# ntnu-arl/aerial_gym_simulator

Hardware: AMD Instinct MI355X
Metric: env-steps/sec at N_envs=8192 per GPU (dynamics-only) (higher is better)
Workload: dtype f32; 1 GPU; base_quadrotor position_setpoint_task, lee_position_control, empty_env, 1 sub-step/step (BASELINE configs[1]); num_envs_per_gpu=8192, num_envs_total=8192, rng=sync-free (device Philox4x32-10)

## Files before the change

### aerial_gym_simulator_amd/csrc/agx_dyn_position_step.h

```cpp
#pragma once

namespace agx {
#ifdef AGX_STEP_STAMPS
constexpr int kStampBlocks = 1024, kStampWords = 8;
__device__ unsigned long long g_step_stamps[kStampBlocks * 2 * kStampWords];
AGX_DEV void step_stamp(int k) {
  const unsigned long long t = k < 6 ? (unsigned long long)clock64() : (unsigned long long)wall_clock64();
  if ((threadIdx.x & 63u) == 0u && blockIdx.x < (unsigned)kStampBlocks)
    g_step_stamps[((size_t)blockIdx.x * 2 + (threadIdx.x >> 6)) * kStampWords + k] = t;
}
#define AGX_STAMP(k) step_stamp(k)
#define AGX_STAMP_ARRIVED(k) do { __builtin_amdgcn_s_waitcnt(0); step_stamp(k); } while (0)
#else
#define AGX_STAMP(k) do { } while (0)
#define AGX_STAMP_ARRIVED(k) do { } while (0)
#endif

AGX_DEV unsigned proof_key(float x) { return x >= 0.0f ? __float_as_uint(x) : 0x7FC00000u; }

__host__ __device__ inline unsigned proof_witness_bit(int episode_len, int reset_on_collision, int steps, float dist, float speed, float dt,
                                                      float vmax, float dv) {
  const int k = episode_len - steps + 1;
  if (k < 1 || k > AGX_PROOF_HORIZON || !(dist == dist) || !(speed == speed)) return 0u;
  bool w = k == 1 || !reset_on_collision;
  if (!w) {
    const float m = (float)(k - 1);
    const float travel = m * dt * fminf(vmax, speed + m * dv);
    w = dist + (travel * 1.01f + 1.0e-3f) < 8.0f;
  }
  return w ? (1u << k) : 0u;
}

template <bool MAX>
AGX_DEV unsigned wave_reduce_dpp(unsigned x) {
#define AGX_RED(ctrl)                                                                        \
  {                                                                                           \
    const unsigned y_ = (unsigned)__builtin_amdgcn_mov_dpp((int)x, (ctrl), 0xF, 0xF, true);   \
    x = MAX ? max(x, y_) : (x | y_);                                                          \
  }
  AGX_RED(0xB1)
  AGX_RED(0x4E)
  AGX_RED(0x124)
  AGX_RED(0x128)
#undef AGX_RED
  const unsigned r0 = (unsigned)__builtin_amdgcn_readlane((int)x, 0), r1 = (unsigned)__builtin_amdgcn_readlane((int)x, 16);
  const unsigned r2 = (unsigned)__builtin_amdgcn_readlane((int)x, 32), r3 = (unsigned)__builtin_amdgcn_readlane((int)x, 48);
  return MAX ? max(max(r0, r1), max(r2, r3)) : ((r0 | r1) | (r2 | r3));
}

AGX_DEV void proof_store_slot(const AgxTaskArgs &T, const AgxEnvBuffers &B, int wb, int nb, bool reset, unsigned horizon, int steps,
                              float dist, float speed) {
  const unsigned ar = wave_reduce_dpp<false>(reset ? 1u : 0u), hz = wave_reduce_dpp<false>(horizon);
  const unsigned ms = wave_reduce_dpp<true>((unsigned)max(steps, 0)), db = wave_reduce_dpp<true>(proof_key(dist));
  const unsigned vb = wave_reduce_dpp<true>(proof_key(speed));
  if ((threadIdx.x & 63u) == 0u) {
    uint4 *slot = reinterpret_cast<uint4 *>(T.proof_slots + ((size_t)(B.step_counter & 1) * nb + wb) * AGX_PROOF_SLOT_WORDS);
    slot[0] = make_uint4(((unsigned)B.step_counter + 1u) & 0x7FFFFFFFu, ar | (T.proof_mode == AGX_STEP_ANY ? 2u : 0u), hz, ms);
    slot[1] = make_uint4(db, vb, 0u, 0u);
  }
}

AGX_DEV void proof_fold_publish(const AgxTaskArgs &T, const AgxEnvBuffers &B, int nb) {
  const int lane = (int)(threadIdx.x & 63u);
  const uint32_t *bank = T.proof_slots + (size_t)((B.step_counter & 1) ^ 1) * nb * AGX_PROOF_SLOT_WORDS;
  unsigned t_and = 0x7FFFFFFFu, t_or = 0u, fl = 0u, hz = 0u, ms = 0u, db = 0u, vb = 0u;
  for (int b = lane; b < nb; b += 64) {
    const uint4 s0 = reinterpret_cast<const uint4 *>(bank + (size_t)b * AGX_PROOF_SLOT_WORDS)[0];
    const uint4 s1 = reinterpret_cast<const uint4 *>(bank + (size_t)b * AGX_PROOF_SLOT_WORDS)[1];
    t_and &= s0.x; t_or |= s0.x; fl |= s0.y; hz |= s0.z;
    ms = max(ms, s0.w); db = max(db, s1.x); vb = max(vb, s1.y);
  }
#pragma unroll
  for (int off = 32; off > 0; off >>= 1) {
    t_and &= (unsigned)__shfl_xor((int)t_and, off);
    t_or |= (unsigned)__shfl_xor((int)t_or, off);
    fl |= (unsigned)__shfl_xor((int)fl, off);
    hz |= (unsigned)__shfl_xor((int)hz, off);
    ms = max(ms, (unsigned)__shfl_xor((int)ms, off));
    db = max(db, (unsigned)__shfl_xor((int)db, off));
    vb = max(vb, (unsigned)__shfl_xor((int)vb, off));
  }
  if (lane != 0) return;
  const unsigned tag = t_and == t_or ? t_or : 0u;
  if (tag != 0u && (fl & 2u) && !(fl & 1u)) atomicAdd(T.proof_violation, 1u);
  uint32_t *h = T.proof_record;
  __hip_atomic_store(h + 7, tag, __ATOMIC_RELAXED, __HIP_MEMORY_SCOPE_SYSTEM);
  __builtin_amdgcn_fence(__ATOMIC_RELEASE, "wavefront");
  __builtin_amdgcn_s_waitcnt(0);
  __hip_atomic_store(h + 1, hz, __ATOMIC_RELAXED, __HIP_MEMORY_SCOPE_SYSTEM);
  __hip_atomic_store(h + 2, ms, __ATOMIC_RELAXED, __HIP_MEMORY_SCOPE_SYSTEM);
  __hip_atomic_store(h + 3, db, __ATOMIC_RELAXED, __HIP_MEMORY_SCOPE_SYSTEM);
  __hip_atomic_store(h + 4, vb, __ATOMIC_RELAXED, __HIP_MEMORY_SCOPE_SYSTEM);
  __hip_atomic_store(h + 5, fl, __ATOMIC_RELAXED, __HIP_MEMORY_SCOPE_SYSTEM);
  __builtin_amdgcn_fence(__ATOMIC_RELEASE, "wavefront");
  __builtin_amdgcn_s_waitcnt(0);
  __hip_atomic_store(h + 0, tag, __ATOMIC_RELAXED, __HIP_MEMORY_SCOPE_SYSTEM);
}

struct StepHandoff {
  float p[64], q[64], v[64], w[64];
  int reset[64];
};
template <int MODE>
AGX_DEV void position_step_quad(const AgxRobotParams &P0, const AgxEnvBuffers &B0, int n, const float *actions_in,
                                const AgxTaskArgs &T0, float *obs, StepHandoff *H) {
  constexpr bool FUSED = MODE != AGX_STEP_TWO;
  const int tid = threadIdx.x;
  AGX_STAMP(0); AGX_STAMP(6);
  AgxRobotParams P = P0;
  AgxEnvBuffers B = B0;
  AgxTaskArgs T = T0;
#define AGX_STEP_WAVE_ARGS(X)                                                                                                        \
  X(B, state) X(B, actions) X(B, prev_actions) X(B, motor_thrust) X(B, motor_kT) X(B, motor_tau_inc) X(B, motor_tau_dec)  \
  X(B, gains) X(B, wrench_cmd) X(B, crashes) X(B, truncations) X(B, sim_steps) X(B, reset_mask) X(B, reset_flag) X(B, flag_parity)    \
  X(B, step_counter) X(B, body_force)                                                                                                  \
  X(P, dt) X(P, dt_over_6) X(P, mass) X(P, min_thrust) X(P, max_thrust) X(P, max_rate) X(P, linear_damping) X(P, angular_damping)     \
  X(P, max_linear_velocity) X(P, max_angular_velocity) X(P, tau_inc_uniform) X(P, tau_dec_uniform)                                    \
  X(T, episode_len) X(T, target) X(T, reward) X(T, proof_slots) X(T, proof_violation) X(T, proof_dv)
  AGX_STEP_WAVE_ARGS(AGX_ARG_READ)
  AGX_ARG_READ(B, derived) AGX_ARG_READ(B, push_world)
  AGX_ARG_READ(P, root_link_mode) AGX_ARG_READ(P, use_rps) AGX_ARG_READ(P, use_discrete_approximation) AGX_ARG_READ(P, integration_rk4)
  AGX_ARG_READ(T, reset_on_collision) AGX_ARG_READ(T, kind) AGX_ARG_READ(T, proof_mode)
  const int grid_blocks = (int)gridDim.x;
  __builtin_amdgcn_sched_barrier(0);
  int env_blocks = grid_blocks - 1;
  int sw = (P_root_link_mode != 0 ? 1 : 0) | (P_use_rps != 0 ? 2 : 0) | (P_use_discrete_approximation != 0 ? 4 : 0) |
           (P_integration_rk4 != 0 ? 8 : 0) | (T_reset_on_collision != 0 ? 16 : 0) | ((T_kind & 0xFF) << 8) | ((T_proof_mode & 0xFF) << 16);
  arg_pin(n); arg_pin(actions_in);
  if (MODE == AGX_STEP_NONE) arg_pin(obs);
  AGX_STEP_WAVE_ARGS(AGX_ARG_PIN)
  if (MODE != AGX_STEP_ANY) { AGX_ARG_PIN(B, derived) }
  if (!FUSED) { AGX_ARG_PIN(B, push_world) }
  arg_pin(env_blocks);
#undef AGX_STEP_WAVE_ARGS
  arg_pin(sw);
  P.root_link_mode = sw & 1; P.use_rps = sw & 2; P.use_discrete_approximation = sw & 4; P.integration_rk4 = sw & 8;
  T.reset_on_collision = sw & 16; T.kind = (sw >> 8) & 0xFF; T.proof_mode = (sw >> 16) & 0xFF;
  const bool proof = T.proof_slots != nullptr;
  if (proof && blockIdx.x == 0) {
    proof_fold_publish(T0, B0, (int)gridDim.x - 1);
    AGX_STAMP(5); AGX_STAMP(7);
    return;
  }
  const int wb = (int)blockIdx.x - (proof ? 1 : 0);
  const int l = tid & 3, l3 = l < 3 ? l : 2;
  const int i = wb * 16 + (tid >> 2);
  const unsigned ol = ((unsigned)l * (unsigned)n + (unsigned)i) * 4u, ol3 = ((unsigned)l3 * (unsigned)n + (unsigned)i) * 4u;
  const bool valid = i < n;
  bool reset = false;
  if (FUSED && wb == 0 && tid == 0) B.reset_flag[B.flag_parity ^ 1] = 0;
  const bool push = !FUSED && wb == 0 && B.push_world > 0;
  uint32_t push_peek = 0u;
  if (__builtin_expect(push, false)) {
    push_publish_previous(B0);
    push_peek = push_wait_peek(B0);
  }
  float p = 0.0f, q = 0.0f, v = 0.0f, w = 0.0f, tgt = 0.0f, vbody = 0.0f, wbody = 0.0f;
  int steps = 0;
  float proof_dist = 0.0f, proof_speed = 0.0f;
  unsigned horizon = 0u;
  float u[1] = {0.0f}, a_in = 0.0f, a_old = 0.0f, fz = 0.0f, torque = 0.0f, dist = 0.0f;
  QuadDerived d{};
  bool crashed = false, trunc = false;
  AGX_STAMP(1);
  if (valid) {
    p = AGX_QAT(B.state, 0, ol3); q = AGX_QAT(B.state, 3, ol); v = AGX_QAT(B.state, 7, ol3); w = AGX_QAT(B.state, 10, ol3);
    u[0] = AGX_QAT(B.motor_thrust, 0, ol);
    float kT[1] = {1.0f}, tinc[1] = {P.tau_inc_uniform}, tdec[1] = {P.tau_dec_uniform};
    if (P.use_rps) kT[0] = AGX_QAT(B.motor_kT, 0, ol);
    if (B.motor_tau_inc) tinc[0] = AGX_QAT(B.motor_tau_inc, 0, ol);
    if (B.motor_tau_dec) tdec[0] = AGX_QAT(B.motor_tau_dec, 0, ol);
    a_in = actions_in[(size_t)i * 4 + l];
    a_old = AGX_QAT(B.actions, 0, ol);
    float kp = P0.gains_uniform[0 + l3], kv = P0.gains_uniform[3 + l3], kr = P0.gains_uniform[6 + l3], kw = P0.gains_uniform[9 + l3];
    if (B.gains) {
      kp = gain_load(&AGX_QAT(B.gains, 0, ol3)); kv = gain_load(&AGX_QAT(B.gains, 3, ol3));
      kr = gain_load(&AGX_QAT(B.gains, 6, ol3)); kw = gain_load(&AGX_QAT(B.gains, 9, ol3));
    }
    const int steps_in = B.sim_steps[i];
    tgt = T.kind == AGX_TASK_POSITION ? AGX_QAT(T.target, 0, ol3) : 0.0f;
    const QuadConsts<4> C = load_quad_consts<4>(P0, P, l, l3);
    AGX_STAMP_ARRIVED(2);

    const float a = clamp_minmax(a_in, -10.0f, 10.0f);
    float sy_sp, cy_sp;
    d = update_states_quad(q, v, w, q4::bc<3>(a), sy_sp, cy_sp);
    const float pe = a - p;
    const float ve = 0.0f - v;
    const float acc = kp * pe + kv * ve;
    const float f = (acc - C.grav) * C.mass;
    fz = quad_thrust_along_body_z(q, f, l);
    const float qd = quad_desired_orientation_pos_vel_sc(f, sy_sp, cy_sp, l);
    torque = quad_body_torque<true>(C, q, qd, d.wbody, 0.0f, kr, kw, l);

    float fb, tb;
    quad_allocate<4>(P, C, l == 2 ? fz : 0.0f, torque, u, kT, tinc, tdec, fb, tb);
    if (B.body_force && l < 3) AGX_QAT(B.body_force, 0, ol) = fb;
    quad_integrate(P, C, p, q, v, w, fb, tb, l);

    steps = steps_in + 1;
    if (T.kind == AGX_TASK_POSITION) {
      const float pe_t = q4::quat_apply(q4::conj(d.qveh), tgt - p);
      dist = q4::norm3(pe_t);
      if (dist > 8.0f) crashed = true;
      trunc = steps > T.episode_len;
      reset = (crashed && T.reset_on_collision) || trunc;
    }
  }
  AGX_STAMP(3);
  if (MODE == AGX_STEP_ANY) {
    H->p[tid] = p; H->q[tid] = q; H->v[tid] = v; H->w[tid] = w;
    H->reset[tid] = reset ? 1 : 0;
    __syncthreads();
  }
  AGX_STAMP(4);
  if (valid) {
    float rew = 0.0f;
    if (T.kind == AGX_TASK_POSITION) {
      const float ex = exp_cw((l == 0 ? -8.0f : -4.0f) * dist * dist);
      const float pos_reward = 3.0f * q4::bc<0>(ex) + 2.0f * q4::bc<1>(ex);
      const float dist_reward = (20.0f - dist) / 40.0f;
      const float axis_z = l == 2 ? 1.0f : 0.0f;
      const float up = q4::bc<2>(q4::quat_rotate(q, axis_z));
      const float tilt = fabsf(1.0f - up);
      const float spin = q4::norm3(d.wbody);
      const float quo = (1.0f / (l == 0 ? 0.1f + tilt * tilt : 1.0f + spin * spin)) * (l == 0 ? 0.2f : 3.0f);
      const float up_reward = q4::bc<0>(quo);
      const float ang_reward = q4::bc<1>(quo);
      float total = pos_reward + dist_reward + pos_reward * (up_reward + ang_reward);
      total = 1.0f * total;
      if (crashed) total = -20.0f;
      rew = total;
      proof_dist = dist;
    }
    if (proof) {
// ... 95 lines not shown
  float tgt = 0.0f;
  AGX_STAMP(1);
  if (valid) {
    steps_in = B.sim_steps[i];
    if (B.episode_count) ep = B.episode_count[i];
    tgt = T.kind == AGX_TASK_POSITION ? AGX_QAT(T.target, 0, ol3) : 0.0f;
  }
  AGX_STAMP_ARRIVED(2);
  const bool early = valid && T.kind == AGX_TASK_POSITION && steps_in + 1 > T.episode_len;
  ResetValues<4> V{};
  if (vote(early) != 0ull) {
    ResetDraws<4> D{};
    wave_reset_draws<4>(R, B.env_index_base + i, ep, early && l == 0, D);
    V = reset_env_values<4>(P, R, D);
  }
  AGX_STAMP(3);
  __syncthreads();
  AGX_STAMP(4);
  float p = H->p[lane], q = H->q[lane], v = H->v[lane], w = H->w[lane];
  const bool mine = H->reset[lane] != 0;
  const bool late = mine && !early;
  if (vote(late) != 0ull) {
    ResetDraws<4> D{};
    wave_reset_draws<4>(R, B.env_index_base + i, ep, late && l == 0, D);
    const ResetValues<4> V2 = reset_env_values<4>(P, R, D);
    if (late) V = V2;
  }
  if (vote(mine) != 0ull) {
    if (mine && l == 0) reset_env_store<4>(P, B, n, R, i, ep, V);
    const EnvState &s = V.s;
    const float npv = q4::by_lane(l3, q4::bc<0>(s.p.x), q4::bc<0>(s.p.y), q4::bc<0>(s.p.z));
    const float nq = q4::by_lane(l, q4::bc<0>(s.q.x), q4::bc<0>(s.q.y), q4::bc<0>(s.q.z), q4::bc<0>(s.q.w));
    const float nv = q4::by_lane(l3, q4::bc<0>(s.v.x), q4::bc<0>(s.v.y), q4::bc<0>(s.v.z));
    const float nw = q4::by_lane(l3, q4::bc<0>(s.w.x), q4::bc<0>(s.w.y), q4::bc<0>(s.w.z));
    p = mine ? npv : p; q = mine ? nq : q; v = mine ? nv : v; w = mine ? nw : w;
  }
  const QuadDerived d2 = update_states_quad(q, v, w);
  if (valid) {
    if (l < 3) {
      AGX_QAT(B.derived, 0, ol) = d2.euler;
      AGX_QAT(B.derived, 7, ol) = d2.vveh;
      AGX_QAT(B.derived, 10, ol) = d2.vbody;
      AGX_QAT(B.derived, 13, ol) = d2.wbody;
    }
    AGX_QAT(B.derived, 3, ol) = d2.qveh;
    float *o = obs + (size_t)i * 13;
    const float e = tgt - p;
    if (l < 3) { o[l] = e; o[7 + l] = d2.vbody; o[10 + l] = d2.wbody; }
    o[3 + l] = q;
  }
  AGX_STAMP(5); AGX_STAMP(7);
}

__global__ void __launch_bounds__(64, 1)
    k_env_step_quad_position(AgxRobotParams P, AgxEnvBuffers B, int n, const float *__restrict__ actions_in, AgxTaskArgs T) {
  position_step_quad<AGX_STEP_TWO>(P, B, n, actions_in, T, nullptr, nullptr);
}

template <int MODE>
__global__ void __launch_bounds__(MODE == AGX_STEP_ANY ? 128 : 64, 1)
    k_position_step_fused(AgxRobotParams P, AgxEnvBuffers B, int n, const float *__restrict__ actions_in, AgxTaskArgs T, AgxResetArgs R,
                          float *__restrict__ obs) {
  if constexpr (MODE == AGX_STEP_ANY) {
    __shared__ StepHandoff H;
    if (__builtin_amdgcn_readfirstlane((int)(threadIdx.x >> 6)) == 0) position_step_quad<MODE>(P, B, n, actions_in, T, obs, &H);
    else position_step_helper(P, B, n, T, R, obs, &H);
  } else {
    position_step_quad<MODE>(P, B, n, actions_in, T, obs, nullptr);
  }
}

#ifdef AGX_STEP_STAMPS
}
extern "C" int agx_debug_step_stamps(unsigned long long *out, int blocks) {
  if (blocks < 0 || blocks > agx::kStampBlocks) return -1;
  return (int)hipMemcpyFromSymbol(out, HIP_SYMBOL(agx::g_step_stamps), sizeof(unsigned long long) * 2 * agx::kStampWords * (size_t)blocks);
}
namespace agx {
#endif
}

extern "C" float agx_step_proof_dv(const AgxRobotParams *P) {
  if (!P || !(P->mass > 0.0f)) return INFINITY;
  const int M = P->num_motors;
  const float *wmap = P->root_link_mode != 0 ? P->alloc : P->wrench_map;
  float col = 0.0f;
  for (int j = 0; j < M; ++j) col += sqrtf(wmap[j] * wmap[j] + wmap[M + j] * wmap[M + j] + wmap[2 * M + j] * wmap[2 * M + j]);
  const float g = sqrtf(P->gravity[0] * P->gravity[0] + P->gravity[1] * P->gravity[1] + P->gravity[2] * P->gravity[2]);
  return (col * fmaxf(fabsf(P->max_thrust), fabsf(P->min_thrust)) / P->mass + g) * P->dt * 1.1f;
}

extern "C" float agx_step_proof_travel(int m, float speed, float dt, float vmax, float dv, int per_env) {
  if (m <= 0) return 0.0f;
  float travel = 0.0f;
  if (per_env) {
    travel = (float)m * dt * fminf(vmax, speed + (float)m * dv);
  } else {
    float v = speed;
    for (int k = 0; k < m; ++k) {
      v = fminf(v + dv, vmax);
      travel += v * dt;
    }
  }
  return travel * 1.01f + 1.0e-3f;
}

extern "C" uint32_t agx_step_proof_witness_bit(int episode_len, int reset_on_collision, int steps, float dist, float speed, float dt,
                                               float max_linear_velocity, float dv) {
  return proof_witness_bit(episode_len, reset_on_collision, steps, dist, speed, dt, max_linear_velocity, dv);
}

extern "C" int agx_step_proof_decide(const uint32_t *record, const AgxStepProofQuery *q, int32_t *reason) {
  int32_t why = AGX_PROOF_PROVED;
  int mode = AGX_STEP_TWO;
  if (!record || !q) {
    why = AGX_PROOF_OFF;
  } else {
    volatile const uint32_t *h = record;
    const uint32_t end = h[0];
    __atomic_thread_fence(__ATOMIC_ACQUIRE);
    const uint32_t hz = h[1], ms = h[2], db = h[3], vb = h[4], fl = h[5];
    __atomic_thread_fence(__ATOMIC_ACQUIRE);
    const uint32_t begin = h[7];
    const uint32_t k = (q->now_tag - end) & 0x7FFFFFFFu;
    float dist, speed;
    memcpy(&dist, &db, 4);
    memcpy(&speed, &vb, 4);
    if (end != begin) why = AGX_PROOF_TORN;
    else if (end == 0u) why = AGX_PROOF_NO_RECORD;
    else if (((end - q->min_tag) & 0x7FFFFFFFu) >= 0x40000000u) why = AGX_PROOF_VOID;
    else if (k == 0u || k > 64u) why = AGX_PROOF_TAG;
    else if (k <= AGX_PROOF_HORIZON && ((hz >> k) & 1u)) mode = AGX_STEP_ANY;
    else if (fl & 1u) why = AGX_PROOF_RESET_NO_WITNESS;
    else if ((int64_t)ms + (int64_t)k > (int64_t)q->episode_len) why = AGX_PROOF_MAY_TRUNCATE;
    else if (q->reset_on_collision && (!(speed == speed) ||
                                       !(dist + agx_step_proof_travel((int)k, speed, q->dt, q->max_linear_velocity, q->dv, 0) < 8.0f)))
      why = AGX_PROOF_MAY_CRASH;
    else mode = AGX_STEP_NONE;
  }
  if (reason) *reason = why;
  return mode;
}

extern "C" int agx_host_record_alloc(size_t bytes, void **out) {
  AGX_REQUIRE(out && bytes > 0 && bytes <= (1u << 20), "bad arguments");
  void *p = nullptr;
  const hipError_t e = hipHostMalloc(&p, bytes, hipHostMallocMapped | hipHostMallocCoherent);
  if (e != hipSuccess) return fail(AGX_E_LAUNCH, "hipHostMalloc(%zu, mapped | coherent): %s", bytes, hipGetErrorString(e));
  memset(p, 0, bytes);
  *out = p;
  return AGX_OK;
}

extern "C" int agx_host_record_free(void *p) {
  if (p) (void)hipHostFree(p);
  return AGX_OK;
}

static int position_step_mode(AgxPositionStepPlan *plan, const AgxTaskArgs &T, hipStream_t stream, bool *slots, int32_t *reason) {
  *slots = false;
  const AgxEnvBuffers *B = plan->buf;
  const AgxRobotParams *P = plan->params;
  if (!option_single_launch_step() || !plan->proof_slots || !plan->proof_record || !plan->proof_violation) {
    *reason = AGX_PROOF_OFF;
    return AGX_STEP_TWO;
  }
  const bool covered = plan->k_substeps == 1 && pick_block(plan->num_envs) == 64 && P->num_motors == 4 &&
                       P->controller == AGX_CTRL_POSITION && T.kind == AGX_TASK_POSITION && quad_kernel_usable(P, B, &T) &&
                       plan->reset->u_state == nullptr && B->episode_count && !B->step_rows[0] && !B->step_rows[1] &&
                       !B->step_signal && B->push_world <= 0 && !B->step_counter_dev && plan->obs && plan->target == T.target;
  if (!covered) {
    *reason = AGX_PROOF_NOT_COVERED;
    return AGX_STEP_TWO;
  }
  if (!plan->captured) {
    hipStreamCaptureStatus cs = hipStreamCaptureStatusNone;
    if (hipStreamIsCapturing(stream, &cs) != hipSuccess || cs != hipStreamCaptureStatusNone) plan->captured = 1;
  }
  if (plan->captured) {
    *reason = AGX_PROOF_CAPTURE;
    return AGX_STEP_TWO;
  }
  *slots = true;
  const int max_lag = plan->max_lag > 0 ? plan->max_lag : 8;
  AgxStepProofQuery Q{};
  Q.now_tag = ((uint32_t)B->step_counter + 1u) & 0x7FFFFFFFu;
  Q.min_tag = plan->proof_min_tag;
  Q.episode_len = T.episode_len;
  Q.reset_on_collision = T.reset_on_collision;
  Q.dt = P->dt;
  Q.max_linear_velocity = P->max_linear_velocity;
  Q.dv = T.proof_dv;
  if (plan->slot_run > max_lag) {
    volatile const uint32_t *h = plan->proof_record;
    uint32_t k = (Q.now_tag - h[0]) & 0x7FFFFFFFu;
    if (h[0] != 0u && k > (uint32_t)max_lag && k <= 64u) {
      const auto t0 = std::chrono::steady_clock::now();
      const auto waited = [&] {
        plan->lag_waits += 1;
        plan->lag_wait_ns += (uint64_t)std::chrono::duration_cast<std::chrono::nanoseconds>(std::chrono::steady_clock::now() - t0).count();
      };
      for (unsigned spin = 1;; ++spin) {
        k = (Q.now_tag - h[0]) & 0x7FFFFFFFu;
        if (k <= (uint32_t)max_lag || k > 64u) break;
        __builtin_ia32_pause();
        if ((spin & 255u) == 0u && std::chrono::steady_clock::now() - t0 > std::chrono::microseconds(2000)) {
          waited();
          *reason = AGX_PROOF_LAG;
          return AGX_STEP_TWO;
        }
      }
      waited();
    }
  }
  return agx_step_proof_decide(plan->proof_record, &Q, reason);
}

extern "C" int agx_position_task_step(AgxPositionStepPlan *plan, const float *actions_in, void *stream) {
  AGX_REQUIRE(plan && plan->params && plan->buf && plan->task && plan->reset, "null plan member");
  AGX_REQUIRE(plan->max_lag == 0 || (plan->max_lag >= 2 && plan->max_lag < AGX_PROOF_HORIZON), "max_lag %d outside 2 .. %d (0: 8)",
              plan->max_lag, AGX_PROOF_HORIZON - 1);
  plan->buf->flag_parity ^= 1;
  if (plan->buf->push_world > 0)
    if (int e = agx_push_advance(plan->buf)) return e;
  AgxTaskArgs T = *plan->task;
  T.proof_slots = nullptr;
  T.proof_record = nullptr;
  T.proof_violation = nullptr;
  T.proof_mode = AGX_STEP_TWO;
  T.proof_dv = agx_step_proof_dv(plan->params);
  bool slots = false;
  int32_t why = AGX_PROOF_OFF;
  const int mode = position_step_mode(plan, T, (hipStream_t)stream, &slots, &why);
  plan->last_mode = mode;
  plan->last_reason = why;
  plan->mode_count[mode] += 1;
  plan->reason_count[why] += 1;
  plan->slot_run = slots ? plan->slot_run + 1 : 0;
  if (slots) {
    T.proof_slots = plan->proof_slots;
    T.proof_record = plan->proof_record;
    T.proof_violation = plan->proof_violation;
    T.proof_mode = mode;
  }
  if (mode != AGX_STEP_TWO) {
    const AgxEnvBuffers *B = plan->buf;
    const int n = plan->num_envs;
    if (int e = check_reset(plan->params, B, n, plan->reset)) return e;
    AGX_REQUIRE(actions_in && B->state && B->derived && B->actions && B->prev_actions && B->motor_thrust && B->crashes && B->truncations &&
                    B->sim_steps && T.target && T.reward,
                "null buffer");
    const dim3 grid(blocks_for(n, 16) + 1);
    if (mode == AGX_STEP_ANY)
      hipLaunchKernelGGL(k_position_step_fused<AGX_STEP_ANY>, grid, dim3(128), 0, (hipStream_t)stream, *plan->params, *B, n, actions_in, T,
                         *plan->reset, plan->obs);
    else
      hipLaunchKernelGGL(k_position_step_fused<AGX_STEP_NONE>, grid, dim3(64), 0, (hipStream_t)stream, *plan->params, *B, n, actions_in, T,
                         *plan->reset, plan->obs);
    return check_launch("agx_position_task_step");
  }
  if (int e = agx_env_step(plan->params, plan->buf, plan->num_envs, actions_in, plan->k_substeps, &T, stream)) return e;
  const uint32_t wait_seq = plan->buf->push_wait_seq;
  plan->buf->push_wait_seq = 0;
  const int rc = agx_post_step_position(plan->params, plan->buf, plan->num_envs, plan->reset, plan->target, plan->obs, stream);
  plan->buf->push_wait_seq = wait_seq;
  return rc;
}
```

### aerial_gym_simulator_amd/csrc/agx_dyn_state.h

```cpp
#pragma once

namespace agx {
#if AGX_DYN_FAST_RCP
AGX_DEV float srcp(float x) {
  float r = __builtin_amdgcn_rcpf(x);
  return fmaf(r, fmaf(-x, r, 1.0f), r);
}
AGX_DEV float fdiv(float a, float b) { return a * srcp(b); }
AGX_DEV float fsqrt(float x) { return __builtin_amdgcn_sqrtf(x); }
#else
AGX_DEV float fdiv(float a, float b) { return a / b; }
AGX_DEV float fsqrt(float x) { return sqrtf(x); }
#endif
AGX_DEV V3 normalized(V3 v) {
  float nv = norm(v);
  return V3{fdiv(v.x, nv), fdiv(v.y, nv), fdiv(v.z, nv)};
}
}

namespace agx {
struct EnvState {
  V3 p;
  Q4 q;
  V3 v, w;
};
struct Derived {
  V3 euler;
  Q4 qveh;
  V3 vveh, vbody, wbody;
};
struct Gains {
  V3 kp, kv, kr, kw;
};
struct Wrench {
  V3 f, t;
};


template <class T>
struct SoaRef {
  static_assert(sizeof(T) == 4, "32-bit elements");
  T *base;
  unsigned col_bytes, lane_bytes;
  AGX_DEV __amdgpu_buffer_rsrc_t rsrc() const {
    return __builtin_amdgcn_make_buffer_rsrc(const_cast<typename std::remove_const<T>::type *>(base), 0, -1, 0x00020000);
  }
  AGX_DEV operator typename std::remove_const<T>::type() const {
    return __builtin_bit_cast(typename std::remove_const<T>::type,
                              __builtin_amdgcn_raw_buffer_load_b32(rsrc(), (int)lane_bytes, (int)col_bytes, 0));
  }
  AGX_DEV void operator=(typename std::remove_const<T>::type v) const {
    __builtin_amdgcn_raw_buffer_store_b32(__builtin_bit_cast(int, v), rsrc(), (int)lane_bytes, (int)col_bytes, 0);
  }
};
template <class T>
AGX_DEV SoaRef<T> soa_at(T *base, int c, int n, int i) {
  return SoaRef<T>{base, (unsigned)c * (unsigned)n * (unsigned)sizeof(T), (unsigned)i * (unsigned)sizeof(T)};
}
#define AGX_AT(p, c) agx::soa_at((p), (c), n, i)
template <class T>
AGX_DEV T &soa_at_off(T *base, int c, int n, unsigned off_bytes) {
  T *col = base + (ptrdiff_t)c * (ptrdiff_t)n;
  return *reinterpret_cast<T *>(reinterpret_cast<char *>(const_cast<typename std::remove_const<T>::type *>(col)) + (size_t)off_bytes);
}
#define AGX_QAT(p, c, off) agx::soa_at_off((p), (c), n, (off))

#define AGX_ARG_READ(S, f) auto S##_##f = S##0 .f;
#define AGX_ARG_READ_N(S, f, N) \
  float S##_##f[N];             \
  _Pragma("unroll") for (int k_ = 0; k_ < N; ++k_) S##_##f[k_] = S##0 .f[k_];
#define AGX_ARG_PIN(S, f) \
  arg_pin(S##_##f);       \
  S.f = S##_##f;
#define AGX_ARG_PIN_N(S, f, N) \
  _Pragma("unroll") for (int k_ = 0; k_ < N; ++k_) { arg_pin(S##_##f[k_]); S.f[k_] = S##_##f[k_]; }
template <class T>
AGX_DEV void arg_pin(T &x) {
  static_assert(sizeof(T) == 4 || sizeof(T) == 8, "one or two scalar registers");
  asm volatile("" : "+s"(x));
}
template <class T>
AGX_DEV void arg_pin(T *&p) {
  typedef T __attribute__((address_space(1))) *global_ptr;
  global_ptr g = (global_ptr)p;
  asm volatile("" : "+s"(g));
  p = (T *)g;
}
AGX_DEV float gain_load(const float *p) { return __hip_atomic_load(p, __ATOMIC_RELAXED, __HIP_MEMORY_SCOPE_WAVEFRONT); }
template <class T, int N>
AGX_DEV void arg_pin(T (&a)[N]) {
#pragma unroll
  for (int k = 0; k < N; ++k) arg_pin(a[k]);
}

AGX_DEV EnvState load_state(const float *__restrict__ s, int n, int i) {
  EnvState e;
  e.p = V3{AGX_AT(s, 0), AGX_AT(s, 1), AGX_AT(s, 2)};
  e.q = Q4{AGX_AT(s, 3), AGX_AT(s, 4), AGX_AT(s, 5), AGX_AT(s, 6)};
  e.v = V3{AGX_AT(s, 7), AGX_AT(s, 8), AGX_AT(s, 9)};
  e.w = V3{AGX_AT(s, 10), AGX_AT(s, 11), AGX_AT(s, 12)};
  return e;
}
AGX_DEV void store_state(float *__restrict__ s, int n, int i, const EnvState &e) {
  AGX_AT(s, 0) = e.p.x; AGX_AT(s, 1) = e.p.y; AGX_AT(s, 2) = e.p.z;
  AGX_AT(s, 3) = e.q.x; AGX_AT(s, 4) = e.q.y; AGX_AT(s, 5) = e.q.z; AGX_AT(s, 6) = e.q.w;
  AGX_AT(s, 7) = e.v.x; AGX_AT(s, 8) = e.v.y; AGX_AT(s, 9) = e.v.z;
  AGX_AT(s, 10) = e.w.x; AGX_AT(s, 11) = e.w.y; AGX_AT(s, 12) = e.w.z;
}
AGX_DEV void store_derived(float *__restrict__ d, int n, int i, const Derived &x) {
  AGX_AT(d, 0) = x.euler.x; AGX_AT(d, 1) = x.euler.y; AGX_AT(d, 2) = x.euler.z;
  AGX_AT(d, 3) = x.qveh.x; AGX_AT(d, 4) = x.qveh.y; AGX_AT(d, 5) = x.qveh.z; AGX_AT(d, 6) = x.qveh.w;
  AGX_AT(d, 7) = x.vveh.x; AGX_AT(d, 8) = x.vveh.y; AGX_AT(d, 9) = x.vveh.z;
  AGX_AT(d, 10) = x.vbody.x; AGX_AT(d, 11) = x.vbody.y; AGX_AT(d, 12) = x.vbody.z;
  AGX_AT(d, 13) = x.wbody.x; AGX_AT(d, 14) = x.wbody.y; AGX_AT(d, 15) = x.wbody.z;
}
AGX_DEV void store_body_velocities(float *__restrict__ d, int n, int i, const Derived &x) {
  AGX_AT(d, 10) = x.vbody.x; AGX_AT(d, 11) = x.vbody.y; AGX_AT(d, 12) = x.vbody.z;
  AGX_AT(d, 13) = x.wbody.x; AGX_AT(d, 14) = x.wbody.y; AGX_AT(d, 15) = x.wbody.z;
}
AGX_DEV Derived load_derived(const float *__restrict__ d, int n, int i) {
// ... 26 lines not shown
```

### aerial_gym_simulator_amd/csrc/agx_dynamics.hip

```cpp
#include "agx_common.h"
#ifndef AGX_DYN_CONTRACT
#define AGX_DYN_CONTRACT 0
#endif
#ifndef AGX_DYN_WAVES
#define AGX_DYN_WAVES 3
#endif
#ifndef AGX_DYN_WAVES_LEAN_LAWS
#define AGX_DYN_WAVES_LEAN_LAWS 4
#endif
#ifndef AGX_DYN_WAVES_LOOP
#define AGX_DYN_WAVES_LOOP 2
#endif
#if AGX_DYN_CONTRACT
#pragma clang fp contract(fast)
#else
#pragma clang fp contract(off)
#endif
#include "agx_device_math.h"
#include "agx_nav_parts.h"
#include "agx_quad_math.h"
#include "agx_rng.h"
#include "agx_step_signal.h"

#include <chrono>
// ... 97 lines not shown
    return EnvStepChoice{ENV_STEP_QUAD_POSITION, 4, AGX_CTRL_POSITION, true, true, 64, blocks_for(n, 16)};
  if (quad_loop_kernel_usable(P, B, n, k))
    return EnvStepChoice{ENV_STEP_QUAD_LOOP, P->num_motors, P->controller, false, true, 64, blocks_for(n, 16)};
  return EnvStepChoice{ENV_STEP_ONE_LANE, P->num_motors, P->controller, k == 1, block == 64, block, blocks_for(n, block)};
}

constexpr size_t kLdsDefaultMax = 64 * 1024;
constexpr size_t kEnvStepLdsMax = (size_t)AGX_MAX_SUBSTEPS * 3 * 256 * sizeof(float);
static_assert(kEnvStepLdsMax <= 160 * 1024, "the sub-step positions of a 256-thread workgroup must fit the CU's 160 KiB of LDS");

template <int M, int CTRL>
static int launch_env_step(const EnvStepChoice &c, size_t lds, hipStream_t stream, const AgxRobotParams &P, const AgxEnvBuffers &B, int n,
                           const float *actions_in, int k, const AgxTaskArgs &T) {
  const auto kernel = c.single ? (c.wide ? k_env_step<M, CTRL, true, true> : k_env_step<M, CTRL, true, false>)
                               : (c.wide ? k_env_step<M, CTRL, false, true> : k_env_step<M, CTRL, false, false>);
  if (lds > kLdsDefaultMax) {
    hipError_t e = hipFuncSetAttribute((const void *)kernel, hipFuncAttributeMaxDynamicSharedMemorySize, (int)kEnvStepLdsMax);
    AGX_REQUIRE(e == hipSuccess, "hipFuncSetAttribute(k_env_step, %zu bytes of LDS): %s", lds, hipGetErrorString(e));
  }
  hipLaunchKernelGGL(kernel, dim3(c.grid), dim3(c.block), lds, stream, P, B, n, actions_in, k, T);
  return AGX_OK;
}

extern "C" int agx_env_step(const AgxRobotParams *P, const AgxEnvBuffers *B, int n, const float *actions_in, int k,
                            const AgxTaskArgs *task, void *stream) {
  if (int e = check_common(P, B, n)) return e;
  AGX_REQUIRE(P != nullptr, "null params");
  AGX_REQUIRE(actions_in != nullptr, "null actions");
  AGX_REQUIRE(k >= 0 && k <= AGX_MAX_SUBSTEPS, "k_substeps out of range: %d", k);
  AGX_REQUIRE(P->controller != AGX_CTRL_WRENCH || k <= 1,
              "external controller (AGX_CTRL_WRENCH): one launch per physics sub-step, the host re-evaluates the controller in between");
  AGX_REQUIRE((B->launch_flags & ~0xFF0F) == 0, "launch_flags: bits 0-3 and the sub-step index in bits 8-15");
  AGX_REQUIRE((B->launch_flags & AGX_LAUNCH_BODY_WRENCH) == 0 || P->controller == AGX_CTRL_WRENCH,
              "AGX_LAUNCH_BODY_WRENCH (external robot) goes with AGX_CTRL_WRENCH: actions_in is a wrench [N][6]");
  AGX_REQUIRE((B->launch_flags & 4) == 0 || ((B->launch_flags & 3) == 0 && P->controller != AGX_CTRL_WRENCH &&
                                             (!task || task->kind != AGX_TASK_NAVIGATION)),
              "AGX_LAUNCH_LEAN needs the fused step of a built-in controller without the navigation reward (it reads the action history)");
  AGX_REQUIRE(B->state && B->derived && B->actions && B->prev_actions && B->motor_thrust && B->crashes && B->truncations &&
                  B->sim_steps,
              "null env buffer");
  AGX_REQUIRE(!P->use_rps || B->motor_kT, "null motor_kT with use_rps");
  AgxTaskArgs T{};
  if (task) T = *task;
  AGX_REQUIRE(T.kind >= AGX_TASK_NONE && T.kind <= AGX_TASK_NAVIGATION, "bad task kind %d", T.kind);
  if (T.kind != AGX_TASK_NONE) {
    AGX_REQUIRE(T.target && T.reward && B->reset_mask && B->reset_flag, "null task buffer");
    AGX_REQUIRE(T.kind != AGX_TASK_NAVIGATION || (T.pos_err && T.prev_pos_err && P->num_actions >= 4), "null navigation buffer");
    AGX_REQUIRE((!T.successes && !T.timeouts && !T.counters) || (T.successes && T.timeouts && T.counters && T.kind == AGX_TASK_NAVIGATION),
                "navigation bookkeeping in the epilogue needs successes, timeouts and counters, and the navigation task kind");
  }
  const EnvStepChoice c = choose_env_step(P, B, n, k, T);
  const dim3 grid(c.grid), block(c.block);
  if (c.family == ENV_STEP_QUAD_POSITION) {
    hipLaunchKernelGGL(k_env_step_quad_position, dim3(c.grid + (T.proof_slots ? 1 : 0)), block, 0, (hipStream_t)stream, *P, *B, n,
                       actions_in, T);
    return check_launch("agx_env_step");
  }
  AGX_REQUIRE(!T.proof_slots && T.proof_mode == AGX_STEP_TWO, "AgxTaskArgs.proof_*: the four-lanes-per-env position kernel only");
  const size_t lds = B->boxes ? (size_t)k * 3 * (c.family == ENV_STEP_QUAD_LOOP ? 16 : c.block) * sizeof(float) : 0;
  if (c.family == ENV_STEP_QUAD_LOOP) {
#define AGX_QUAD_LOOP(M_, C_)                                                                                                          \
  if (c.M == M_ && c.ctrl == C_)                                                                                                       \
    hipLaunchKernelGGL((k_env_step_quad_loop<M_, C_>), grid, block, lds, (hipStream_t)stream, *P, *B, n, actions_in, k, T);
    AGX_QUAD_LOOP(4, AGX_CTRL_POSITION)
    AGX_QUAD_LOOP(4, AGX_CTRL_VELOCITY)
    AGX_QUAD_LOOP(4, AGX_CTRL_ATTITUDE)
    AGX_QUAD_LOOP(4, AGX_CTRL_RATES)
    AGX_QUAD_LOOP(4, AGX_CTRL_ACCELERATION)
    AGX_QUAD_LOOP(4, AGX_CTRL_VEL_STEERING)
    AGX_QUAD_LOOP(8, AGX_CTRL_POSITION)
    AGX_QUAD_LOOP(8, AGX_CTRL_VELOCITY)
    AGX_QUAD_LOOP(8, AGX_CTRL_FULLY_ACTUATED)
#undef AGX_QUAD_LOOP
    return check_launch("agx_env_step");
  }
  AGX_REQUIRE(lds <= kEnvStepLdsMax, "agx_env_step needs %zu bytes of LDS (> %zu)", lds, kEnvStepLdsMax);
  AGX_DISPATCH_M(c.M, AGX_DISPATCH_CTRL(c.ctrl, if (int e = launch_env_step<kM, kC>(c, lds, (hipStream_t)stream, *P, *B, n, actions_in, k, T)) return e));
  return check_launch("agx_env_step");
}

extern "C" int agx_env_step_kernel(const AgxRobotParams *P, const AgxEnvBuffers *B, int n, int k, const AgxTaskArgs *task, char *out,
                                   int cap) {
  AGX_REQUIRE(P && B && out && cap > 0 && n > 0, "bad arguments");
  AgxTaskArgs T{};
  if (task) T = *task;
  const EnvStepChoice c = choose_env_step(P, B, n, k, T);
  const int threads = c.grid * c.block;
  if (c.family == ENV_STEP_QUAD_POSITION)
    snprintf(out, (size_t)cap, "k_env_step_quad_position_%d", threads);
  else if (c.family == ENV_STEP_QUAD_LOOP)
    snprintf(out, (size_t)cap, "k_env_step_quad_loop<%d,%d>_%d", c.M, c.ctrl, threads);
  else
    snprintf(out, (size_t)cap, "k_env_step<%d,%d,%s,%s>_%d", c.M, c.ctrl, c.single ? "true" : "false", c.wide ? "true" : "false", threads);
  return AGX_OK;
}

extern "C" int agx_dynamics_substeps(const AgxRobotParams *P, const AgxEnvBuffers *B, int n, const float *actions_in,
                                     int k, void *stream) {
  return agx_env_step(P, B, n, actions_in, k, nullptr, stream);
}

extern "C" int agx_push_advance(AgxEnvBuffers *b) {
  AGX_REQUIRE(b && b->push_world > 0 && b->push_world <= 8 && b->push_slots >= 5 && b->push_base && b->push_slice_bytes > 0,
              "agx_push_advance: peer push is not bound (or fewer than 5 receive slots)");
  b->push_pub_seq = b->push_seq;
  b->push_pub_index = b->push_flag_index;
  const uint32_t seq = ++b->push_seq;
  const int slot = (int)((seq - 1u) % (uint32_t)b->push_slots);
// ... 11 lines not shown
```

Measured before the change: 1.019 billion env-steps/s.

## Pack hot step pointers into a cache-line-aligned kernarg head and issue loads early

Adds a 128-byte aligned AgxStepHead at the start of the kernel argument segment. It holds the pointers, n and flags needed for the first global loads. The kernel reads this head first and issues the per-env state, thrust, gain and target loads, using branch-free pointer substitution so nothing waits on flag checks. Only after that does it read the rest of the parameters directly from the kernarg segment through address-space-4 pointers. The aim is to shorten the dependency chain from kernel start to the first memory request in a latency-bound tiny kernel, at the cost of extra speculative loads and a more complicated argument layout.

```diff
diff --git a/aerial_gym_simulator_amd/csrc/agx_dyn_position_step.h b/aerial_gym_simulator_amd/csrc/agx_dyn_position_step.h
--- a/aerial_gym_simulator_amd/csrc/agx_dyn_position_step.h
+++ b/aerial_gym_simulator_amd/csrc/agx_dyn_position_step.h
@@ -60,9 +60,9 @@
   }
 }
 
-AGX_DEV void proof_fold_publish(const AgxTaskArgs &T, const AgxEnvBuffers &B, int nb) {
+AGX_DEV void proof_fold_publish(const uint32_t *slots, uint32_t *record, uint32_t *violation, int step_counter, int nb) {
   const int lane = (int)(threadIdx.x & 63u);
-  const uint32_t *bank = T.proof_slots + (size_t)((B.step_counter & 1) ^ 1) * nb * AGX_PROOF_SLOT_WORDS;
+  const uint32_t *bank = slots + (size_t)((step_counter & 1) ^ 1) * nb * AGX_PROOF_SLOT_WORDS;
   unsigned t_and = 0x7FFFFFFFu, t_or = 0u, fl = 0u, hz = 0u, ms = 0u, db = 0u, vb = 0u;
   for (int b = lane; b < nb; b += 64) {
     const uint4 s0 = reinterpret_cast<const uint4 *>(bank + (size_t)b * AGX_PROOF_SLOT_WORDS)[0];
@@ -82,8 +82,8 @@
   }
   if (lane != 0) return;
   const unsigned tag = t_and == t_or ? t_or : 0u;
-  if (tag != 0u && (fl & 2u) && !(fl & 1u)) atomicAdd(T.proof_violation, 1u);
-  uint32_t *h = T.proof_record;
+  if (tag != 0u && (fl & 2u) && !(fl & 1u)) atomicAdd(violation, 1u);
+  uint32_t *h = record;
   __hip_atomic_store(h + 7, tag, __ATOMIC_RELAXED, __HIP_MEMORY_SCOPE_SYSTEM);
   __builtin_amdgcn_fence(__ATOMIC_RELEASE, "wavefront");
   __builtin_amdgcn_s_waitcnt(0);
@@ -101,60 +101,57 @@
   float p[64], q[64], v[64], w[64];
   int reset[64];
 };
-template <int MODE>
-AGX_DEV void position_step_quad(const AgxRobotParams &P0, const AgxEnvBuffers &B0, int n, const float *actions_in,
-                                const AgxTaskArgs &T0, float *obs, StepHandoff *H) {
+template <int MODE, class AT>
+AGX_DEV void position_step_quad(const AgxStepHead &A0, const AgxRobotParams &P0, const AgxEnvBuffers &B0, const AgxTaskArgs &T0,
+                                StepHandoff *H) {
   constexpr bool FUSED = MODE != AGX_STEP_TWO;
   const int tid = threadIdx.x;
   AGX_STAMP(0); AGX_STAMP(6);
+  AGX_ARG_READ(A, state) AGX_ARG_READ(A, motor_thrust) AGX_ARG_READ(A, actions) AGX_ARG_READ(A, sim_steps) AGX_ARG_READ(A, motor_kT)
+  AGX_ARG_READ(A, motor_tau_inc) AGX_ARG_READ(A, motor_tau_dec) AGX_ARG_READ(A, gains) AGX_ARG_READ(A, actions_in) AGX_ARG_READ(A, target)
+  AGX_ARG_READ(A, n) AGX_ARG_READ(A, flags)
+  const int l = tid & 3, l3 = l < 3 ? l : 2;
+  const unsigned il = (unsigned)tid >> 2;
+  __builtin_amdgcn_sched_barrier(0);
+  arg_pin(A_state); arg_pin(A_motor_thrust); arg_pin(A_actions); arg_pin(A_sim_steps); arg_pin(A_motor_kT); arg_pin(A_motor_tau_inc);
+  arg_pin(A_motor_tau_dec); arg_pin(A_gains); arg_pin(A_actions_in); arg_pin(A_target); arg_pin(A_n); arg_pin(A_flags);
   AgxRobotParams P = P0;
   AgxEnvBuffers B = B0;
   AgxTaskArgs T = T0;
+  B.state = A_state; B.motor_thrust = A_motor_thrust; B.actions = A_actions; B.sim_steps = A_sim_steps; B.motor_kT = A_motor_kT;
+  B.motor_tau_inc = A_motor_tau_inc; B.motor_tau_dec = A_motor_tau_dec; B.gains = A_gains; T.target = A_target;
+  const int n = A_n;
+  const float *actions_in = A_actions_in;
+  arg_seg seg = (arg_seg)__builtin_amdgcn_kernarg_segment_ptr();
+  asm volatile("" : "+s"(seg));
+  const auto *Pc = (const AgxRobotParams __attribute__((address_space(4))) *)(seg + offsetof(AT, P));
+  const auto *Bc = (const AgxEnvBuffers __attribute__((address_space(4))) *)(seg + offsetof(AT, B));
+  const auto *Tc = (const AgxTaskArgs __attribute__((address_space(4))) *)(seg + offsetof(AT, T));
 #define AGX_STEP_WAVE_ARGS(X)                                                                                                        \
-  X(B, state) X(B, actions) X(B, prev_actions) X(B, motor_thrust) X(B, motor_kT) X(B, motor_tau_inc) X(B, motor_tau_dec)  \
-  X(B, gains) X(B, wrench_cmd) X(B, crashes) X(B, truncations) X(B, sim_steps) X(B, reset_mask) X(B, reset_flag) X(B, flag_parity)    \
+  X(B, prev_actions) X(B, wrench_cmd) X(B, crashes) X(B, truncations) X(B, reset_mask) X(B, reset_flag) X(B, flag_parity)             \
   X(B, step_counter) X(B, body_force)                                                                                                  \
   X(P, dt) X(P, dt_over_6) X(P, mass) X(P, min_thrust) X(P, max_thrust) X(P, max_rate) X(P, linear_damping) X(P, angular_damping)     \
   X(P, max_linear_velocity) X(P, max_angular_velocity) X(P, tau_inc_uniform) X(P, tau_dec_uniform)                                    \
-  X(T, episode_len) X(T, target) X(T, reward) X(T, proof_slots) X(T, proof_violation) X(T, proof_dv)
-  AGX_STEP_WAVE_ARGS(AGX_ARG_READ)
-  AGX_ARG_READ(B, derived) AGX_ARG_READ(B, push_world)
-  AGX_ARG_READ(P, root_link_mode) AGX_ARG_READ(P, use_rps) AGX_ARG_READ(P, use_discrete_approximation) AGX_ARG_READ(P, integration_rk4)
-  AGX_ARG_READ(T, reset_on_collision) AGX_ARG_READ(T, kind) AGX_ARG_READ(T, proof_mode)
-  const int grid_blocks = (int)gridDim.x;
+  X(T, episode_len) X(T, reward) X(T, proof_slots) X(T, proof_violation) X(T, proof_dv)
+  AGX_STEP_WAVE_ARGS(AGX_ARG_READ_AT)
+  AGX_ARG_READ_AT(B, derived) AGX_ARG_READ_AT(B, push_world) AGX_ARG_READ_AT(T, proof_record)
+  AGX_ARG_READ_AT(P, use_discrete_approximation) AGX_ARG_READ_AT(P, integration_rk4) AGX_ARG_READ_AT(T, reset_on_collision)
+  AGX_ARG_READ_AT(T, proof_mode)
+  float *obs = nullptr;
+  if constexpr (MODE == AGX_STEP_NONE) obs = *(float *const __attribute__((address_space(4))) *)(seg + offsetof(AT, obs));
   __builtin_amdgcn_sched_barrier(0);
-  int env_blocks = grid_blocks - 1;
-  int sw = (P_root_link_mode != 0 ? 1 : 0) | (P_use_rps != 0 ? 2 : 0) | (P_use_discrete_approximation != 0 ? 4 : 0) |
-           (P_integration_rk4 != 0 ? 8 : 0) | (T_reset_on_collision != 0 ? 16 : 0) | ((T_kind & 0xFF) << 8) | ((T_proof_mode & 0xFF) << 16);
-  arg_pin(n); arg_pin(actions_in);
-  if (MODE == AGX_STEP_NONE) arg_pin(obs);
-  AGX_STEP_WAVE_ARGS(AGX_ARG_PIN)
-  if (MODE != AGX_STEP_ANY) { AGX_ARG_PIN(B, derived) }
-  if (!FUSED) { AGX_ARG_PIN(B, push_world) }
-  arg_pin(env_blocks);
-#undef AGX_STEP_WAVE_ARGS
-  arg_pin(sw);
-  P.root_link_mode = sw & 1; P.use_rps = sw & 2; P.use_discrete_approximation = sw & 4; P.integration_rk4 = sw & 8;
-  T.reset_on_collision = sw & 16; T.kind = (sw >> 8) & 0xFF; T.proof_mode = (sw >> 16) & 0xFF;
-  const bool proof = T.proof_slots != nullptr;
-  if (proof && blockIdx.x == 0) {
-    proof_fold_publish(T0, B0, (int)gridDim.x - 1);
+  const bool proof = (A_flags & kHeadSlots) != 0u;
+  const int env_blocks = (n + 15) >> 4;
+  if (__builtin_expect(proof && blockIdx.x == 0, false)) {
+    proof_fold_publish(T_proof_slots, T_proof_record, T_proof_violation, B_step_counter, env_blocks);
     AGX_STAMP(5); AGX_STAMP(7);
     return;
   }
   const int wb = (int)blockIdx.x - (proof ? 1 : 0);
-  const int l = tid & 3, l3 = l < 3 ? l : 2;
-  const int i = wb * 16 + (tid >> 2);
+  const int i = wb * 16 + (int)il;
   const unsigned ol = ((unsigned)l * (unsigned)n + (unsigned)i) * 4u, ol3 = ((unsigned)l3 * (unsigned)n + (unsigned)i) * 4u;
   const bool valid = i < n;
   bool reset = false;
-  if (FUSED && wb == 0 && tid == 0) B.reset_flag[B.flag_parity ^ 1] = 0;
-  const bool push = !FUSED && wb == 0 && B.push_world > 0;
-  uint32_t push_peek = 0u;
-  if (__builtin_expect(push, false)) {
-    push_publish_previous(B0);
-    push_peek = push_wait_peek(B0);
-  }
   float p = 0.0f, q = 0.0f, v = 0.0f, w = 0.0f, tgt = 0.0f, vbody = 0.0f, wbody = 0.0f;
   int steps = 0;
   float proof_dist = 0.0f, proof_speed = 0.0f;
@@ -162,25 +159,57 @@
   float u[1] = {0.0f}, a_in = 0.0f, a_old = 0.0f, fz = 0.0f, torque = 0.0f, dist = 0.0f;
   QuadDerived d{};
   bool crashed = false, trunc = false;
+  float kT_in, tinc_in, tdec_in, kp, kv, kr, kw, ku[4];
+  int steps_in;
+  QuadConsts<4> C;
   AGX_STAMP(1);
   if (valid) {
-    p = AGX_QAT(B.state, 0, ol3); q = AGX_QAT(B.state, 3, ol); v = AGX_QAT(B.state, 7, ol3); w = AGX_QAT(B.state, 10, ol3);
-    u[0] = AGX_QAT(B.motor_thrust, 0, ol);
-    float kT[1] = {1.0f}, tinc[1] = {P.tau_inc_uniform}, tdec[1] = {P.tau_dec_uniform};
-    if (P.use_rps) kT[0] = AGX_QAT(B.motor_kT, 0, ol);
-    if (B.motor_tau_inc) tinc[0] = AGX_QAT(B.motor_tau_inc, 0, ol);
-    if (B.motor_tau_dec) tdec[0] = AGX_QAT(B.motor_tau_dec, 0, ol);
-    a_in = actions_in[(size_t)i * 4 + l];
-    a_old = AGX_QAT(B.actions, 0, ol);
-    float kp = P0.gains_uniform[0 + l3], kv = P0.gains_uniform[3 + l3], kr = P0.gains_uniform[6 + l3], kw = P0.gains_uniform[9 + l3];
-    if (B.gains) {
-      kp = gain_load(&AGX_QAT(B.gains, 0, ol3)); kv = gain_load(&AGX_QAT(B.gains, 3, ol3));
-      kr = gain_load(&AGX_QAT(B.gains, 6, ol3)); kw = gain_load(&AGX_QAT(B.gains, 9, ol3));
-    }
-    const int steps_in = B.sim_steps[i];
-    tgt = T.kind == AGX_TASK_POSITION ? AGX_QAT(T.target, 0, ol3) : 0.0f;
-    const QuadConsts<4> C = load_quad_consts<4>(P0, P, l, l3);
-    AGX_STAMP_ARRIVED(2);
+#define AGX_LD(base, c, off) (*reinterpret_cast<const float *>(reinterpret_cast<const char *>(base) + (size_t)((unsigned)(c) * (unsigned)n * 4u) + (size_t)(off)))
+    p = AGX_LD(B.state, 0, ol3); q = AGX_LD(B.state, 3, ol); v = AGX_LD(B.state, 7, ol3); w = AGX_LD(B.state, 10, ol3);
+    u[0] = AGX_LD(B.motor_thrust, 0, ol);
+    const bool use_rps = (A_flags & kHeadUseRps) != 0u, position = ((A_flags >> 8) & 0xFFu) == (unsigned)AGX_TASK_POSITION;
+    kT_in = AGX_LD(use_rps ? B.motor_kT : B.motor_thrust, 0, ol);
+    tinc_in = AGX_LD(B.motor_tau_inc ? B.motor_tau_inc : B.motor_thrust, 0, ol);
+    tdec_in = AGX_LD(B.motor_tau_dec ? B.motor_tau_dec : B.motor_thrust, 0, ol);
+    a_in = *reinterpret_cast<const float *>(reinterpret_cast<const char *>(actions_in) + (size_t)((unsigned)i * 16u + (unsigned)l * 4u));
+    a_old = AGX_LD(B.actions, 0, ol);
+    const float ku0 = P0.gains_uniform[0 + l3], ku1 = P0.gains_uniform[3 + l3], ku2 = P0.gains_uniform[6 + l3], ku3 = P0.gains_uniform[9 + l3];
+    const float *gsrc = B.gains ? B.gains : B.state;
+    const float kg0 = gain_load(&AGX_LD(gsrc, 0, ol3)), kg1 = gain_load(&AGX_LD(gsrc, 3, ol3));
+    const float kg2 = gain_load(&AGX_LD(gsrc, 6, ol3)), kg3 = gain_load(&AGX_LD(gsrc, 9, ol3));
+    steps_in = *reinterpret_cast<const int *>(reinterpret_cast<const char *>(B.sim_steps) + (size_t)((unsigned)i * 4u));
+    const float tgt_in = AGX_LD(position ? T.target : B.state, 0, ol3);
+#undef AGX_LD
+    P.root_link_mode = (int)(A_flags & kHeadRootLink);
+    C = load_quad_consts<4>(P0, P, l, l3);
+    kp = kg0; kv = kg1; kr = kg2; kw = kg3; ku[0] = ku0; ku[1] = ku1; ku[2] = ku2; ku[3] = ku3;
+    tgt = tgt_in;
+  }
+  __builtin_amdgcn_sched_barrier(0);
+  int sw = (int)(A_flags & (kHeadRootLink | kHeadUseRps | 0xFF00u)) | (P_use_discrete_approximation != 0 ? 4 : 0) |
+           (P_integration_rk4 != 0 ? 8 : 0) | (T_reset_on_collision != 0 ? 16 : 0) | ((T_proof_mode & 0xFF) << 16);
+  if (MODE == AGX_STEP_NONE) arg_pin(obs);
+  AGX_STEP_WAVE_ARGS(AGX_ARG_PIN)
+  if (MODE != AGX_STEP_ANY) { AGX_ARG_PIN(B, derived) }
+  if (!FUSED) { AGX_ARG_PIN(B, push_world) }
+#undef AGX_STEP_WAVE_ARGS
+  arg_pin(sw);
+  P.root_link_mode = sw & 1; P.use_rps = sw & 2; P.use_discrete_approximation = sw & 4; P.integration_rk4 = sw & 8;
+  T.reset_on_collision = sw & 16; T.kind = (sw >> 8) & 0xFF; T.proof_mode = (sw >> 16) & 0xFF;
+  if (FUSED && wb == 0 && tid == 0) B.reset_flag[B.flag_parity ^ 1] = 0;
+  const bool push = !FUSED && wb == 0 && B.push_world > 0;
+  uint32_t push_peek = 0u;
+  if (__builtin_expect(push, false)) {
+    push_publish_previous(B0);
+    push_peek = push_wait_peek(B0);
+  }
+  AGX_STAMP_ARRIVED(2);
+  if (valid) {
+    C.mass = P.mass; C.dt = P.dt;
+    if (!B.gains) { kp = ku[0]; kv = ku[1]; kr = ku[2]; kw = ku[3]; }
+    if (T.kind != AGX_TASK_POSITION) tgt = 0.0f;
+    const float kT[1] = {P.use_rps ? kT_in : 1.0f}, tinc[1] = {B.motor_tau_inc ? tinc_in : P.tau_inc_uniform};
+    const float tdec[1] = {B.motor_tau_dec ? tdec_in : P.tau_dec_uniform};
 
     const float a = clamp_minmax(a_in, -10.0f, 10.0f);
     float sy_sp, cy_sp;
@@ -382,21 +411,21 @@
   AGX_STAMP(5); AGX_STAMP(7);
 }
 
-__global__ void __launch_bounds__(64, 1)
-    k_env_step_quad_position(AgxRobotParams P, AgxEnvBuffers B, int n, const float *__restrict__ actions_in, AgxTaskArgs T) {
-  position_step_quad<AGX_STEP_TWO>(P, B, n, actions_in, T, nullptr, nullptr);
+struct KernelArgsTwo { AgxStepHead A; AgxRobotParams P; AgxEnvBuffers B; AgxTaskArgs T; };
+struct KernelArgsFused { AgxStepHead A; AgxRobotParams P; AgxEnvBuffers B; int n; AgxTaskArgs T; AgxResetArgs R; float *obs; };
+__global__ void __launch_bounds__(64, 1) k_env_step_quad_position(AgxStepHead A, AgxRobotParams P, AgxEnvBuffers B, AgxTaskArgs T) {
+  position_step_quad<AGX_STEP_TWO, KernelArgsTwo>(A, P, B, T, nullptr);
 }
 
 template <int MODE>
 __global__ void __launch_bounds__(MODE == AGX_STEP_ANY ? 128 : 64, 1)
-    k_position_step_fused(AgxRobotParams P, AgxEnvBuffers B, int n, const float *__restrict__ actions_in, AgxTaskArgs T, AgxResetArgs R,
-                          float *__restrict__ obs) {
+    k_position_step_fused(AgxStepHead A, AgxRobotParams P, AgxEnvBuffers B, int n, AgxTaskArgs T, AgxResetArgs R, float *__restrict__ obs) {
   if constexpr (MODE == AGX_STEP_ANY) {
     __shared__ StepHandoff H;
-    if (__builtin_amdgcn_readfirstlane((int)(threadIdx.x >> 6)) == 0) position_step_quad<MODE>(P, B, n, actions_in, T, obs, &H);
+    if (__builtin_amdgcn_readfirstlane((int)(threadIdx.x >> 6)) == 0) position_step_quad<MODE, KernelArgsFused>(A, P, B, T, &H);
     else position_step_helper(P, B, n, T, R, obs, &H);
   } else {
-    position_step_quad<MODE>(P, B, n, actions_in, T, obs, nullptr);
+    position_step_quad<MODE, KernelArgsFused>(A, P, B, T, nullptr);
   }
 }
 
@@ -485,6 +514,16 @@
 extern "C" int agx_host_record_free(void *p) {
   if (p) (void)hipHostFree(p);
   return AGX_OK;
+}
+
+static AgxStepHead step_head(const AgxRobotParams &P, const AgxEnvBuffers &B, int n, const float *actions_in, const AgxTaskArgs &T) {
+  AgxStepHead A{};
+  A.state = B.state; A.motor_thrust = B.motor_thrust; A.actions = B.actions; A.sim_steps = B.sim_steps;
+  A.motor_kT = B.motor_kT; A.motor_tau_inc = B.motor_tau_inc; A.motor_tau_dec = B.motor_tau_dec; A.gains = B.gains;
+  A.actions_in = actions_in; A.target = T.target; A.n = n;
+  A.flags = (P.root_link_mode != 0 ? kHeadRootLink : 0u) | (P.use_rps != 0 ? kHeadUseRps : 0u) | (T.proof_slots ? kHeadSlots : 0u) |
+            (((uint32_t)T.kind & 0xFFu) << 8);
+  return A;
 }
 
 static int position_step_mode(AgxPositionStepPlan *plan, const AgxTaskArgs &T, hipStream_t stream, bool *slots, int32_t *reason) {
@@ -581,11 +620,12 @@
                     B->sim_steps && T.target && T.reward,
                 "null buffer");
     const dim3 grid(blocks_for(n, 16) + 1);
+    const AgxStepHead A = step_head(*plan->params, *B, n, actions_in, T);
     if (mode == AGX_STEP_ANY)
-      hipLaunchKernelGGL(k_position_step_fused<AGX_STEP_ANY>, grid, dim3(128), 0, (hipStream_t)stream, *plan->params, *B, n, actions_in, T,
+      hipLaunchKernelGGL(k_position_step_fused<AGX_STEP_ANY>, grid, dim3(128), 0, (hipStream_t)stream, A, *plan->params, *B, n, T,
                          *plan->reset, plan->obs);
     else
-      hipLaunchKernelGGL(k_position_step_fused<AGX_STEP_NONE>, grid, dim3(64), 0, (hipStream_t)stream, *plan->params, *B, n, actions_in, T,
+      hipLaunchKernelGGL(k_position_step_fused<AGX_STEP_NONE>, grid, dim3(64), 0, (hipStream_t)stream, A, *plan->params, *B, n, T,
                          *plan->reset, plan->obs);
     return check_launch("agx_position_task_step");
   }
diff --git a/aerial_gym_simulator_amd/csrc/agx_dyn_state.h b/aerial_gym_simulator_amd/csrc/agx_dyn_state.h
--- a/aerial_gym_simulator_amd/csrc/agx_dyn_state.h
+++ b/aerial_gym_simulator_amd/csrc/agx_dyn_state.h
@@ -65,7 +65,19 @@
 }
 #define AGX_QAT(p, c, off) agx::soa_at_off((p), (c), n, (off))
 
+struct alignas(64) AgxStepHead {
+  float *state, *motor_thrust, *actions;
+  int32_t *sim_steps;
+  float *motor_kT, *motor_tau_inc, *motor_tau_dec, *gains;
+  const float *actions_in, *target;
+  int32_t n;
+  uint32_t flags;
+};
+static_assert(sizeof(AgxStepHead) == 128 && alignof(AgxStepHead) == 64, "two lines at the start of the segment");
+constexpr uint32_t kHeadRootLink = 1u, kHeadUseRps = 2u, kHeadSlots = 32u;
 #define AGX_ARG_READ(S, f) auto S##_##f = S##0 .f;
+typedef const char __attribute__((address_space(4))) *arg_seg;
+#define AGX_ARG_READ_AT(S, f) auto S##_##f = S##c->f;
 #define AGX_ARG_READ_N(S, f, N) \
   float S##_##f[N];             \
   _Pragma("unroll") for (int k_ = 0; k_ < N; ++k_) S##_##f[k_] = S##0 .f[k_];
diff --git a/aerial_gym_simulator_amd/csrc/agx_dynamics.hip b/aerial_gym_simulator_amd/csrc/agx_dynamics.hip
--- a/aerial_gym_simulator_amd/csrc/agx_dynamics.hip
+++ b/aerial_gym_simulator_amd/csrc/agx_dynamics.hip
@@ -173,8 +173,8 @@
   const EnvStepChoice c = choose_env_step(P, B, n, k, T);
   const dim3 grid(c.grid), block(c.block);
   if (c.family == ENV_STEP_QUAD_POSITION) {
-    hipLaunchKernelGGL(k_env_step_quad_position, dim3(c.grid + (T.proof_slots ? 1 : 0)), block, 0, (hipStream_t)stream, *P, *B, n,
-                       actions_in, T);
+    hipLaunchKernelGGL(k_env_step_quad_position, dim3(c.grid + (T.proof_slots ? 1 : 0)), block, 0, (hipStream_t)stream,
+                       step_head(*P, *B, n, actions_in, T), *P, *B, T);
     return check_launch("agx_env_step");
   }
   AGX_REQUIRE(!T.proof_slots && T.proof_mode == AGX_STEP_TWO, "AgxTaskArgs.proof_*: the four-lanes-per-env position kernel only");
```

Measured after the change: 972.8 million env-steps/s. 4.5% lower.
